# jhollowed/PyTEMDiags

Hardware: AMD Instinct MI355X
Metric: grid-points/sec through full TEM pipeline (ncol*nlev*nt) (higher is better)
Workload: dtype f64; 1 GPU; ne120 (777602 cols) x 72 lev x 30 snapshots per GPU, L=50, 1-degree zonal grid (M=180), ten GM16 Table-A1 outputs; ncol=777602, nlev=72, nt=30, sweeps=latitude-class, single sweep, mirror_paired_sweeps=True

## Files before the change

### include/temx.h

```cpp
#ifndef TEMX_H
#define TEMX_H

#include <stdint.h>

#ifdef __cplusplus
extern "C" {
#endif

typedef struct temx_plan temx_plan;

enum { TEMX_F64 = 0, TEMX_F32 = 1 };

enum {
  TEMX_OK = 0,
  TEMX_EINVAL = -1,
  TEMX_EHIP = -2,
  TEMX_ENOMEM = -3,
  TEMX_ERANK = -4,
  TEMX_ESTATE = -5,
  TEMX_EUNSUPPORTED = -6,
  TEMX_EINTERNAL = -7
};

enum {
  TEMX_DEFER_FINALIZE = 1,
  TEMX_NO_SYMMETRY = 2,
  TEMX_NO_CLASSES = 4,
  TEMX_NO_QR = 8,
  TEMX_LAT_TOL_F32 = 16
};

enum {
  TEMX_OPT_FORM = 1,
  TEMX_OPT_OS_MAP = 2,
  TEMX_OPT_OP_MAP = 3,
  TEMX_OPT_OS_SUBSAMPLE = 4,
  TEMX_OPT_TRACER_ONE_PASS = 5,
  TEMX_OPT_SINGLE_SWEEP_MIN_GROUPS = 6,
  TEMX_OPT_OS_CONTRACT = 7,
  TEMX_OPT_MISSING = 8,
  TEMX_OPT_MIN_COVERAGE = 9,
  TEMX_OPT_MISSING_WEIGHT = 10,
  TEMX_OPT_LAT_BINS = 12,
  TEMX_OPT_BIN_DEGREE = 13,
  TEMX_OPT_OS_SYNC = 11
};
enum {
  TEMX_FORM_AUTO = -1,
  TEMX_FORM_TWO_PASS = 0,
  TEMX_FORM_CLASS_SUMS = 1,
  TEMX_FORM_SINGLE_SWEEP = 2,
  TEMX_FORM_NO_SINGLE_SWEEP = 3,
  TEMX_FORM_MASKED = 4,
  TEMX_FORM_BINNED = 5
};

enum {
  TEMX_MAT_Y0 = 0,
  TEMX_MAT_Y0P = 1,
  TEMX_MAT_GRAM = 2,
  TEMX_MAT_GINV = 3,
  TEMX_MAT_Y0INV = 4,
  TEMX_MAT_GRAM2 = 5,
  TEMX_MAT_GX = 6,
  TEMX_MAT_GSUB = 7,
  TEMX_MAT_COVERAGE = 8
};
// ... 137 lines not shown
```

### pytemdiags_amd/_lib.py

```python
from __future__ import annotations

import ctypes as C
import os

_HERE = os.path.dirname(os.path.abspath(__file__))
LIB_PATH = os.environ.get("TEMX_LIB") or os.path.join(_HERE, "libtemx.so")

ABI_VERSION = 402
F64, F32 = 0, 1
DEFER_FINALIZE = 1
NO_SYMMETRY = 2
NO_CLASSES = 4
NO_QR = 8
LAT_TOL_F32 = 16
MAT_Y0, MAT_Y0P, MAT_GRAM, MAT_GINV, MAT_Y0INV, MAT_GRAM2, MAT_GX, MAT_GSUB = 0, 1, 2, 3, 4, 5, 6, 7
MAT_COVERAGE = 8
OPT_FORM, OPT_OS_MAP, OPT_OP_MAP, OPT_OS_SUBSAMPLE, OPT_TRACER_ONE_PASS, OPT_SINGLE_SWEEP_MIN_GROUPS, OPT_OS_CONTRACT = 1, 2, 3, 4, 5, 6, 7
OPT_MISSING, OPT_MIN_COVERAGE, OPT_MISSING_WEIGHT = 8, 9, 10
OPT_OS_SYNC = 11
OPT_LAT_BINS, OPT_BIN_DEGREE = 12, 13
LAT_BINS_ALLOWED = (128, 256, 512, 1024, 2048)
LAT_BINS_DEFAULT = 512
MISSING_MODES = {"raise": 0, "mask": 1}
FORM_AUTO, FORM_TWO_PASS, FORM_CLASS_SUMS, FORM_SINGLE_SWEEP, FORM_NO_SINGLE_SWEEP = -1, 0, 1, 2, 3
FORM_MASKED = 4
FORM_BINNED = 5
FORM_NAMES = {FORM_TWO_PASS: "two-pass", FORM_CLASS_SUMS: "class-sums", FORM_SINGLE_SWEEP: "single-sweep",
              FORM_MASKED: "masked", FORM_BINNED: "binned"}
FORMS = {"auto": FORM_AUTO, "two-pass": FORM_TWO_PASS, "class-sums": FORM_CLASS_SUMS,
         "single-sweep": FORM_SINGLE_SWEEP, "no-single-sweep": FORM_NO_SINGLE_SWEEP}

RESULT_NAMES = ("vtem", "omegatem", "wtem", "psitem", "epfy", "epfz", "epdiv",
                "utendepfd", "utendvtem", "utendwtem")
ZONAL_NAMES = ("ub", "vb", "thetab", "wapb", "upvpb", "upwappb", "vptpb", "dub_dp", "dthetab_dp",
               "ubcoslat", "dubcoslat_dlat", "psi", "psicoslat", "dpsicoslat_dlat", "dpsi_dp",
               "int_vbdp")
EDDY_NAMES = ("up", "vp", "thetap", "wapp", "upvp", "upwapp", "vptp")
TRACER_RESULT_NAMES = ("etfy", "etfz", "etdiv", "qtendetfd", "qtendvtem", "qtendwtem")
TRACER_ZONAL_NAMES = ("qb", "qpvpb", "qpwappb", "dqb_dp", "qbcoslat", "dqbcoslat_dlat")
TRACER_EDDY_NAMES = ("qp", "qpvp", "qpwapp")

ERRORS = {0: "TEMX_OK", -1: "TEMX_EINVAL", -2: "TEMX_EHIP", -3: "TEMX_ENOMEM", -4: "TEMX_ERANK",
          -5: "TEMX_ESTATE", -6: "TEMX_EUNSUPPORTED", -7: "TEMX_EINTERNAL"}
# ... 123 lines not shown
```

### pytemdiags_amd/csrc/kernels.hpp

```cpp
#pragma once
#include <hip/hip_runtime.h>
#include <stdint.h>

#include <type_traits>

#define TEMX_MFMA4(a, b, c) __builtin_amdgcn_mfma_f64_4x4x4f64((a), (b), (c), 0, 0, 0)

namespace temx {

template <int NF>
struct FieldPtrs {
  const void* p[NF];
};

struct EddyOut {
  double* p[7];
};

template <int KMAX>
__device__ __forceinline__ void basis_row(double xv, int K, const double* __restrict__ norm,
                                          const double* __restrict__ T, double* q) {
  double pm1 = 1.0, pc = xv;
  for (int l = 0; l < K; ++l) {
    double P;
// ... 220 lines not shown
#pragma unroll
    for (int j = 0; j < 16; ++j) t += sh[j][e];
    if (addend != nullptr) t += addend[idx];
    B[slice_index(map, idx)] = t;
    if (!(fabs(t) <= 1.79769313486231570815e308)) atomicOr(flag, 1);
  }
}

template <int NS>
__global__ void __launch_bounds__(256)
reduce_partials_flat_kernel(const double* __restrict__ partial, int nsplit, int64_t stride, int64_t n,
                            const double* __restrict__ addend, double* __restrict__ B, int* __restrict__ flag,
                            SliceMap map) {
  const int64_t idx = (int64_t)blockIdx.x * 256 + threadIdx.x;
  if (idx >= n) return;
  double v[NS];
#pragma unroll
  for (int sp = 0; sp < NS; ++sp) v[sp] = partial[(int64_t)(sp < nsplit ? sp : 0) * stride + idx];
  double t = 0.0;
#pragma unroll
  for (int sp = 0; sp < NS; ++sp) t += sp < nsplit ? v[sp] : 0.0;
  if (addend != nullptr) t += addend[idx];
  B[slice_index(map, idx)] = t;
  if (!(fabs(t) <= 1.79769313486231570815e308)) atomicOr(flag, 1);
}

__global__ void __launch_bounds__(256)
reduce_rows_kernel(const double* __restrict__ partial, int nsplit, int64_t stride, int nf, int rows_in, int rows,
                   int64_t D, double* __restrict__ out, int* __restrict__ flag) {
  const int64_t idx = (int64_t)blockIdx.x * 256 + threadIdx.x;
  const int64_t per = (int64_t)rows * D;
  if (idx >= per * nf) return;
  const int64_t f = idx / per, rem = idx - f * per;
  const double* src = partial + f * rows_in * D + rem;
  double t = 0.0;
  for (int sp = 0; sp < nsplit; ++sp) t += src[(int64_t)sp * stride];
  out[idx] = t;
  if (!(fabs(t) <= 1.79769313486231570815e308)) atomicOr(flag, 1);
}
__global__ void __launch_bounds__(256)
reduce_rows_wide_kernel(const double* __restrict__ partial, int nsplit, int64_t stride, int nf, int rows_in, int rows,
                        int64_t D, double* __restrict__ out, int* __restrict__ flag) {
  __shared__ double sh[16][17];
  const int e = threadIdx.x & 15, sl = threadIdx.x >> 4;
  const int64_t idx = (int64_t)blockIdx.x * 16 + e;
  const int64_t per = (int64_t)rows * D;
// ... 747 lines not shown
```

### pytemdiags_amd/csrc/kernels_op2.hpp

```cpp
#pragma once
#include "kernels_op.hpp"

namespace temx {

template <int NA, int NB>
struct OpwSlot {
  double sd[2][NA][64];
  double y[NB * 16];
};

template <int TBS, int NA>
__device__ __forceinline__ void opw_round(const OpwSlot<NA, 2 * TBS>* slots, int par, int t0, int nbw,
                                          uint32_t yoff, int lane, double (&acc)[NA][(TBS + 1) / 2]) {
  asm volatile("s_waitcnt lgkmcnt(0)\n\ts_barrier" ::: "memory");
#pragma unroll
  for (int j = 0; j < 4; ++j) {
    double b[NA];
#pragma unroll
    for (int f = 0; f < NA; ++f) b[f] = slots[j].sd[par][f][lane];
#pragma unroll
    for (int tl = 0; tl < (TBS + 1) / 2; ++tl)
      if (tl < nbw) {
        const double ya = slots[j].y[(t0 + tl) * 16 + yoff];
#pragma unroll
// ... 937 lines not shown
    }
    if (hfail != 0 && lane == 0) atomicOr(hstat, hfail);
  }
  if (left > 0) {
    const int first = (b1 - b0) & (NCH - 1);
    static_for<NCH>([&](auto cc) __attribute__((always_inline)) {
      if (((decltype(cc)::value - first) & (NCH - 1)) < left) pending_chunk(cc);
    });
  }
  if (dvalid) {
#pragma unroll
    for (int f = 0; f < NFX; ++f)
#pragma unroll
      for (int t = 0; t < NBX; ++t) {
        const int l = symx_harm<TBX>(t, g);
        if (l < (pp != nullptr ? KX : K4)) px[(((int64_t)split * NFX + f) * KX + l) * D + d] = ax[f][t];
      }
#pragma unroll
    for (int k = 0; k < NP; ++k)
#pragma unroll
      for (int t = 0; t < 2 * TBS; ++t) {
        const int l = sym_harm<TBS>(t, g);
        if (pp != nullptr && l < K) pp[(((int64_t)split * NP + k) * K + l) * D + d] = k < NPR ? apr[k < NPR ? k : 0][t] : apl[((k < NPR ? 0 : k - NPR) * 2 * TBS + t) * 64];
      }
  }
}

#ifndef TEMX_OS2_STAGGER
#define TEMX_OS2_STAGGER 0
#endif
#ifndef TEMX_OS2_ACC32
#define TEMX_OS2_ACC32 1
#endif
template <typename T, int TBS, int TBX, int NBR, int PD, int KIND = 0>
__global__ void __launch_bounds__(512, 1)
sweep_os2_kernel(FieldPtrs<4> fp, int64_t D, int K, int KX, const double* __restrict__ ycx,
                 const int4* __restrict__ crowN, const int4* __restrict__ crowS,
                 const int* __restrict__ gfirstN, const int* __restrict__ gfirstS, const int2* __restrict__ csplit,
                 const double* __restrict__ colscale, const double* __restrict__ rho, int K4,
                 double* __restrict__ px, double* __restrict__ pp, int nsplit, int ndt) {
  using KD = OsKind<KIND>;
  constexpr int NF = KD::NF, NFX = KD::NFX, NP = KD::NP;
  constexpr int NBX = 2 * TBX;
  constexpr int YE = NBX * 16;
  constexpr int MB = CLS_MB;
  constexpr int NCH = 2;
// ... 500 lines not shown
}

__global__ void __launch_bounds__(256)
os_ref_solve_kernel(const double* __restrict__ As, int KX , int KR, int64_t D,
                    const double* __restrict__ Gsinv, double* __restrict__ rho) {
  __shared__ double sg[16 * 16];
  const int f = blockIdx.y;
  for (int i = threadIdx.x; i < KR * KR; i += blockDim.x) sg[i] = Gsinv[i];
  __syncthreads();
  const int64_t d = blockIdx.x * (int64_t)(blockDim.x / 16) + (threadIdx.x & 15);
  const int l = threadIdx.x >> 4;
  if (d >= D || l >= KR) return;
  const double* a = As + (int64_t)f * KX * D + d;
  double v0 = 0.0, v1 = 0.0;
  int m = 0;
  for (; m + 2 <= KR; m += 2) {
    v0 += sg[l * KR + m] * a[(int64_t)m * D];
    v1 += sg[l * KR + m + 1] * a[(int64_t)(m + 1) * D];
  }
  if (m < KR) v0 += sg[l * KR + m] * a[(int64_t)m * D];
  rho[((int64_t)f * KR + l) * D + d] = v0 + v1;
}

constexpr int OSC = 4;
constexpr int OSR = 256 / OSC;

__device__ __forceinline__ void os_stage(double* dst, const double* __restrict__ src, int n, int tid) {
  for (int i = tid; i < n; i += 256) dst[i] = src[i];
}

__host__ __device__ inline size_t os_contract_lds(int K, int KX, int NQ) {
  const size_t big = (size_t)NQ * KX > (size_t)2 * K * K ? (size_t)NQ * KX : (size_t)2 * K * K;
  return ((size_t)4 * KX + 8 * K + 8 * NQ + 3 * KX + 3 * K) * OSC + big;
}

struct OsFields {
  const double* A[4];
  const double* rho[4];
};

template <int KIND>
__global__ void __launch_bounds__(256)
os_contract_kernel(OsFields in, const double* __restrict__ Pp,
                   int K, int KX, int KR, int NQ, int64_t D, const double* __restrict__ Tm,
                   const double* __restrict__ G2inv, const double* __restrict__ G, const double* __restrict__ Gx,
                   const double* __restrict__ Yq, const double* __restrict__ wq2, double* __restrict__ B4,
// ... 144 lines not shown
```

### pytemdiags_amd/csrc/temx.hip

```cpp
#include "../../include/temx.h"
#include "../../include/temx_vert.h"
#include "../../include/temx_layout.h"
#include "../../include/temx_ingest.h"
#include "../../include/temx_clim.h"
#include "../../include/temx_mtracer.h"
#include "../../include/temx_nclim.h"
#include "../../include/temx_gclim.h"
#include "../include/temx_mgclim.h"
#include "../include/temx_wave.h"
#include "../include/temx_tfilt.h"

#include <hip/hip_runtime.h>

#include <algorithm>
#include <cmath>
#include <cstdarg>
#include <cstdio>
#include <cstdlib>
#include <cstring>
#include <map>
#include <mutex>
#include <new>
#include <stdexcept>
#include <string>
// ... 125 lines not shown
  std::vector<int> gbatch0;
  DevBuf crow, ycls;
  std::map<int, DevBuf> csplits;
  Split sp_cproj4, sp_cproj1, sp_ceddy, sp_cflux;
  bool os_built = false, os_on = false;
  bool os_valid = false;
  DevBuf Axq, rho_t;
  int TBX = 0, KX = 0, KR = 0, NQ = 0;
  std::vector<double> h_xc, h_cnt;
  std::vector<int> h_crow;
  std::vector<int> sgbatch0;
  int64_t sgroups = 0, sbatches = 0;
  DevBuf ycx, ycx_s, crow_s, rho, rho0, gaunt , wq2, Gx, Gsinv, Ax , Axs ;
  std::vector<double> h_G_own;
  std::vector<double> h_Gx_own;
  std::vector<double> h_Gx, h_Gs;
  std::vector<double> h_T, h_Ginv, h_G, h_Yq;
  DevBuf oscblk, osAt, osAb, osAtq, osAbq, Bqp;
  OscMats osc{};
  bool osc_lds = false;
  int opt_os_contract = -1;
  bool os_barrier = false;
  int opt_os_sync = -1;
  int os_keep = 32;
  int64_t tD = 0, tnt = 0, tt0 = 0;
  int opt_form = -1, opt_os_map = -1, opt_op_map = -1, opt_tracer_one_pass = -1, opt_single_sweep_min_groups = -1;
  bool os_tile = false, op_tile = false;
  bool no_qr = false;
  DevBuf side_crow[2][2], side_gfirst[2][2];
  std::map<int, DevBuf> csplits_s;
  Split sp_os, sp_os_s;
  Split sp_copw;
  bool lcls = false, lone = false, xb_valid = false;
  DevBuf ycls_l, pbuf;
  int64_t ycls_lstride = 0;
  Split sp_lflux;
  bool onepass = false, op_valid = false;
  bool c4_valid = false;
  DevBuf csum, ccnt;
  DevBuf Pq;
  DevBuf csq, Pq2;
  bool tq_valid = false;
  DevBuf partial;
  DevBuf opB, opC;
  int opt_missing = 0, opt_min_cov = 500, opt_miss_w = 10;
  bool miss_built = false;
// ... 168 lines not shown
}

static int launch_reduce(temx_plan* pl, const double* partial, int nsplit, int64_t n, double* B,
                         hipStream_t st, int64_t stride = -1, const double* addend = nullptr,
                         const SliceMap& map = SliceMap(), int* flag = nullptr) {
  if (stride < 0) stride = n;
  if (flag == nullptr) flag = static_cast<int*>(pl->flag.p);
  if (nsplit <= 16 && n >= 32768) {
    const dim3 grid((unsigned)((n + 255) / 256));
    if (nsplit <= 2)
      hipLaunchKernelGGL(reduce_partials_flat_kernel<2>, grid, dim3(256), 0, st, partial, nsplit, stride, n, addend, B, flag, map);
    else if (nsplit <= 4)
      hipLaunchKernelGGL(reduce_partials_flat_kernel<4>, grid, dim3(256), 0, st, partial, nsplit, stride, n, addend, B, flag, map);
    else if (nsplit <= 8)
      hipLaunchKernelGGL(reduce_partials_flat_kernel<8>, grid, dim3(256), 0, st, partial, nsplit, stride, n, addend, B, flag, map);
    else
      hipLaunchKernelGGL(reduce_partials_flat_kernel<16>, grid, dim3(256), 0, st, partial, nsplit, stride, n, addend, B, flag, map);
    HIPCHK(hipGetLastError());
    return TEMX_OK;
  }
  const int64_t blocks = (n + 15) / 16;
  hipLaunchKernelGGL(reduce_partials_kernel, dim3((unsigned)blocks), dim3(256), 0, st, partial, nsplit, stride, n,
                     addend, B, flag, map);
  HIPCHK(hipGetLastError());
  return TEMX_OK;
}

static int launch_reduce_rows(temx_plan* pl, const double* partial, int nsplit, int64_t stride, int nf, int rows_in,
                              int rows, int64_t D, double* out, hipStream_t st) {
  const int64_t n = (int64_t)nf * rows * D;
  if (nsplit > 16)
    hipLaunchKernelGGL(reduce_rows_wide_kernel, dim3((unsigned)((n + 15) / 16)), dim3(256), 0, st, partial, nsplit, stride,
                       nf, rows_in, rows, D, out, static_cast<int*>(pl->flag.p));
  else
    hipLaunchKernelGGL(reduce_rows_kernel, dim3((unsigned)((n + 255) / 256)), dim3(256), 0, st, partial, nsplit, stride,
                       nf, rows_in, rows, D, out, static_cast<int*>(pl->flag.p));
  HIPCHK(hipGetLastError());
  return TEMX_OK;
}

static int launch_solve(temx_plan* pl, const double* B, int NF, int64_t D, double* C, double* Xb,
                        hipStream_t st) {
  if (pl->K <= 64) {
    const int nmb = (pl->M + 3) / 4;
    const int gx = (int)(((D + 15) / 16 + 3) / 4);
    int mbs = SOLVE_MB;
// ... 472 lines not shown
          static_cast<const int*>(pl->side_gfirst[si][0].p), static_cast<const int*>(pl->side_gfirst[si][1].p),
          cuts, pl->colscale.d(), rho, pl->KR, px, pp, sp.nsplit, sp.ndt);
    }
    constexpr size_t lds = sweep_osr_lds(TBSv, TBXv, KD::NF, KD::NP, KD::NPR, DF);
    static_assert(lds <= 163840, "the single sweep's workgroup fits the LDS of a compute unit");
    auto go = [&](auto handoff) {
      return launch_lds<sweep_osr_kernel<double, TBSv, TBXv, NBR, 2, KIND, decltype(handoff)::value>>(pl->device, grid,
          block, lds, st, fp, pl->D, pl->K, pl->KX, sub ? pl->ycx_s.d() : pl->ycx.d(),
          static_cast<const int4*>(sub ? pl->crow_s.p : pl->crow.p), cuts, pl->colscale.d(), rho, pl->KR, px, pp, sp.nsplit,
          sp.ndt, static_cast<int*>(pl->flag.p) + 1);
    };
    return pl->os_barrier ? go(Int<0>{}) : go(Int<1>{});
  });
  return listed ? rc : fail(TEMX_EUNSUPPORTED, "single-sweep form: no instantiation for L = %d", pl->L);
}

template <int KIND>
static int launch_sweep_os(temx_plan* pl, const FieldPtrs<4>& fp, int dtype, bool sub, const double* rho, double* partial,
                           const Split& sp, hipStream_t st) {
  return dtype == TEMX_F64 ? launch_sweep_os_t<double, KIND>(pl, fp, sub, rho, partial, sp, st)
                           : launch_sweep_os_t<float, KIND>(pl, fp, sub, rho, partial, sp, st);
}

static bool os_supported(const temx_plan* pl) {
  return os_supported(pl->cls, pl->large, pl->weighted, pl->qbasis, !pl->h_crow.empty(), pl->TBS, pl->L);
}

static bool os_active(const temx_plan* pl, int dtype) {
  (void)dtype;
  return pl->os_on;
}

static void set_tail(temx_plan* pl, int64_t t0, int64_t nts) {
  if (pl->tt0 != t0 || pl->tnt != nts) pl->c4_valid = pl->os_valid = pl->op_valid = pl->tq_valid = pl->xb_valid = false;
  pl->tt0 = t0;
  pl->tnt = nts;
  pl->tD = (int64_t)pl->nlev * nts;
}
static inline bool tail_is_whole(const temx_plan* pl) { return pl->tt0 == 0 && pl->tnt == pl->nt; }

static int tem_stage3_impl(temx_plan* pl, const double* B3, double* results, double* zonal, hipStream_t st);
static int tem_epilogue(temx_plan* pl, double* results, double* zonal, hipStream_t st);
static int bin_project_op(temx_plan* pl, const void* A, int dtype, int64_t D, double* B, hipStream_t st);
static int bin_zonal_mean(temx_plan* pl, const void* A, int dtype, int64_t D, double* out, int native, hipStream_t st);
static int miss_check(const temx_plan* pl);
static int miss_zonal_mean(temx_plan* pl, const void* A, int dtype, int64_t D, double* out, int native, hipStream_t st);
// ... 10 lines not shown
  return m;
}

template <int NBK>
static int launch_osc_t(temx_plan* pl, const OscFieldsIn& fin, int nf, int nout, double* Bf, double* At, double* ab,
                        const OscPairsIn& pin, int np, double* Bp, int64_t Dt, hipStream_t st) {
  const unsigned gx = (unsigned)((Dt + 15) / 16);
  hipLaunchKernelGGL((osc_fields_kernel<NBK>), dim3(gx, nf, 2), dim3(OSC_W * 64), (size_t)osc_fields_lds(NBK) * 8, st, fin, pl->osc, pl->K,
                     pl->KX, pl->KR, pl->NQ, Dt, nout, Bf, At, ab, pl->D, (int)pl->tnt, (int)pl->nt, (int)pl->tt0);
  HIPCHK(hipGetLastError());
  hipLaunchKernelGGL((osc_pairs_kernel<NBK>), dim3(gx, np), dim3(OSC_W * 64), (size_t)osc_pairs_lds(NBK) * 8, st, pin, pl->osc, pl->wq2.d(),
                     pl->K, pl->KX, pl->NQ, Dt, Bp);
  HIPCHK(hipGetLastError());
  return TEMX_OK;
}
static int launch_osc(temx_plan* pl, const OscFieldsIn& fin, int nf, int nout, double* Bf, double* At, double* ab,
                      const OscPairsIn& pin, int np, double* Bp, int64_t Dt, hipStream_t st) {
  if (pl->TB == 13 && pl->TBX == 13) return launch_osc_t<13>(pl, fin, nf, nout, Bf, At, ab, pin, np, Bp, Dt, st);
  if (pl->TB == 8 && pl->TBX == 8) return launch_osc_t<8>(pl, fin, nf, nout, Bf, At, ab, pin, np, Bp, Dt, st);
  if (pl->TB == 4 && pl->TBX == 4) return launch_osc_t<4>(pl, fin, nf, nout, Bf, At, ab, pin, np, Bp, Dt, st);
  return fail(TEMX_EUNSUPPORTED, "single-sweep contraction: no instantiation for L = %d", pl->L);
}

static int os_prepass(temx_plan* pl, const FieldPtrs<4>& fp, int dtype, double* As, hipStream_t st) {
  int rc;
  const int64_t D = pl->D, KD4 = (int64_t)4 * pl->KX * D;
  pl->op_valid = pl->c4_valid = pl->tq_valid = pl->os_valid = false;
  if ((rc = launch_sweep_os<0>(pl, fp, dtype, true, pl->rho0.d(), pl->partial.d(), pl->sp_os_s, st))) return rc;
  return launch_reduce_rows(pl, pl->partial.d(), pl->sp_os_s.nsplit, KD4, 4, pl->KX, pl->KR, D, As, st);
}

static int os_sweep(temx_plan* pl, const FieldPtrs<4>& fp, int dtype, const double* As, int nsl, double* proj, hipStream_t st) {
  int rc;
  const int64_t D = pl->D;
  const int64_t KD4 = (int64_t)4 * pl->KX * D, KD3 = (int64_t)3 * pl->K * D;
  pl->op_valid = pl->c4_valid = pl->tq_valid = pl->os_valid = false;
  hipLaunchKernelGGL(os_ref_solve_kernel, dim3((unsigned)((D + 15) / 16), 4), dim3(256), 0, st, As, pl->KR, pl->KR, D,
                     pl->Gsinv.d(), pl->rho.d());
  HIPCHK(hipGetLastError());
  TimedLaunch tl{};
  time_begin(pl, 0, st, tl);
  rc = launch_sweep_os<0>(pl, fp, dtype, false, pl->rho.d(), pl->partial.d(), pl->sp_os, st);
  time_end(pl, 0, st, tl);
  if (rc) return rc;
  const int64_t rows = (int64_t)4 * pl->KX + 3 * pl->K;
  if ((rc = launch_reduce(pl, pl->partial.d(), pl->sp_os.nsplit, KD4, proj, st, -1, nullptr, slice_map(pl, nsl, rows, 0)))) return rc;
  return launch_reduce(pl, pl->partial.d() + (int64_t)pl->sp_os.nsplit * KD4, pl->sp_os.nsplit, KD3, nsl > 1 ? proj : proj + KD4, st, -1,
                       nullptr, slice_map(pl, nsl, rows, (int64_t)4 * pl->KX));
}

static int os_tail(temx_plan* pl, const double* proj_s, int64_t t0, int64_t nts, double* results, double* zonal, hipStream_t st) {
  int rc;
  set_tail(pl, t0, nts);
  const int64_t Dt = pl->tD;
  const int64_t rows = (int64_t)4 * pl->KX + 3 * pl->K;
  if (proj_s != pl->Ax.d())
    HIPCHK(hipMemcpyAsync(pl->Ax.p, proj_s, (size_t)rows * Dt * 8, hipMemcpyDeviceToDevice, st));
  {
    TimedLaunch t2{};
    time_begin(pl, 1, st, t2);
    const size_t lds = os_contract_lds(pl->K, pl->KX, pl->NQ) * 8;
    const double* Pp = pl->Ax.d() + (int64_t)4 * pl->KX * Dt;
    if (pl->osc_lds) {
      OsFields in;
      for (int f = 0; f < 4; ++f) {
        in.A[f] = pl->Ax.d() + (int64_t)f * pl->KX * Dt;
        in.rho[f] = pl->rho.d() + (int64_t)f * pl->KR * pl->D;
      }
// ... 9 lines not shown
      for (int f = 0; f < 4; ++f) {
        fin.A[f] = pl->Ax.d() + (int64_t)f * pl->KX * Dt;
        fin.rho[f] = pl->rho.d() + (int64_t)f * pl->KR * pl->D;
      }
      for (int k = 0; k < 3; ++k) {
        pin.At_a[k] = pl->osAt.d() + KD::pa(k) * QD; pin.At_b[k] = pl->osAt.d() + KD::pb(k) * QD;
        pin.ab_a[k] = pl->osAb.d() + KD::pa(k) * QD; pin.ab_b[k] = pl->osAb.d() + KD::pb(k) * QD;
        pin.P[k] = Pp + (int64_t)k * pl->K * Dt;
      }
      if ((rc = launch_osc(pl, fin, 4, 4, pl->B4.d(), pl->osAt.d(), pl->osAb.d(), pin, 3, pl->B3.d(), Dt, st))) return rc;
    }
    time_end(pl, 1, st, t2);
  }
  if ((rc = launch_solve(pl, pl->B4.d(), 4, Dt, pl->C4.d(), pl->zb.d(), st))) return rc;
  if ((rc = tem_stage3_impl(pl, pl->B3.d(), results, zonal, st))) return rc;
  pl->c4_valid = true;
  pl->os_valid = true;
  return TEMX_OK;
}

static int tem_run_os(temx_plan* pl, const FieldPtrs<4>& fp, int dtype, double* results, double* zonal, void* stream) {
  hipStream_t st = S_(stream);
  int rc;
  if ((rc = os_prepass(pl, fp, dtype, pl->Axs.d(), st))) return rc;
  if ((rc = os_sweep(pl, fp, dtype, pl->Axs.d(), 1, pl->Ax.d(), st))) return rc;
  return os_tail(pl, pl->Ax.d(), 0, pl->nt, results, zonal, st);
}

static int tracer_ws(temx_plan* pl);

static int tracer_os_ws(temx_plan* pl, int nq) {
  const TracerOsWs w = tracer_os_ws_layout(tem_dims(pl), nq, pl->KX, pl->KR, pl->NQ);
  int rc;
  if ((rc = tracer_ws(pl))) return rc;
  if ((rc = pl->Axq.ensure(w.Axq))) return rc;
  if ((rc = pl->osAtq.ensure(w.osAtq))) return rc;
  if ((rc = pl->osAbq.ensure(w.osAbq))) return rc;
  if ((rc = pl->Bqp.ensure(w.Bqp))) return rc;
  return pl->rho_t.ensure(w.rho_t);
}

static int tracer_os_prepass(temx_plan* pl, int nq, const FieldPtrs<4>& fp, int dtype, double* Asq, hipStream_t st) {
  int rc;
  const int64_t D = pl->D;
  if ((rc = tracer_os_ws(pl, nq))) return rc;
  pl->tq_valid = false;
  rc = nq == 2 ? launch_sweep_os<3>(pl, fp, dtype, true, pl->rho0.d(), pl->partial.d(), pl->sp_os_s, st)
               : launch_sweep_os<1>(pl, fp, dtype, true, pl->rho0.d(), pl->partial.d(), pl->sp_os_s, st);
// ... 1225 lines not shown
      break;
    case TEMX_OPT_MISSING_WEIGHT:
      if (value < 4 || value > 14) return fail(TEMX_EINVAL, "TEMX_OPT_MISSING_WEIGHT: tau = 10^-value, value in 4..14, got %d", value);
      pl->opt_miss_w = value;
      break;
    case TEMX_OPT_OS_SYNC:
      if (value != 0 && value != 1) return fail(TEMX_EINVAL, "TEMX_OPT_OS_SYNC: 0 (flags) or 1 (barriers), got %d", value);
      pl->opt_os_sync = value;
      break;
    case TEMX_OPT_LAT_BINS: {
      const int B = value == -1 ? BIN_DEFAULT : value;
      if (B != 0) {
        if (!bin_count_ok(B)) return fail(TEMX_EINVAL, "TEMX_OPT_LAT_BINS: 0 (off), -1 (default, %d) or one of 128, 256, 512, 1024, 2048, got %d", BIN_DEFAULT, value);
        if (int rc = bin_check(pl)) return rc;
        if (bin_degree(pl->L, B) == 0)
          return fail(TEMX_EINVAL, "TEMX_OPT_LAT_BINS: (L, B) = (%d, %d): no Chebyshev degree up to %d keeps the basis rows to %.0e; use more bins",
                      pl->L, B, BIN_MAX_DEGREE, BIN_BOUND);
      }
      pl->opt_lat_bins = B;
      pl->bin_J = B ? bin_degree(pl->L, B) : 0;
      break;
    }
    case TEMX_OPT_BIN_DEGREE: return fail(TEMX_EINVAL, "TEMX_OPT_BIN_DEGREE is chosen by the library (read it with temx_plan_option)");
    default: return fail(TEMX_EINVAL, "unknown option %d", option);
  }
  pl->tem = false;
  return TEMX_OK;
} TEMX_CATCH

int temx_plan_option(const temx_plan* pl, int option) try {
  if (!pl) return -1;
  switch (option) {
    case TEMX_OPT_FORM:
      if (miss_mode(pl)) return TEMX_FORM_MASKED;
      if (bin_mode(pl)) return TEMX_FORM_BINNED;
      return pl->os_on ? TEMX_FORM_SINGLE_SWEEP : ((pl->cls && pl->onepass) || (pl->lcls && pl->lone) ? TEMX_FORM_CLASS_SUMS : TEMX_FORM_TWO_PASS);
    case TEMX_OPT_OS_MAP: return tile_map(pl->opt_os_map, "TEMX_OS_MAP") ? 1 : 0;
    case TEMX_OPT_OP_MAP: return tile_map(pl->opt_op_map, "TEMX_OP_MAP") ? 1 : 0;
    case TEMX_OPT_TRACER_ONE_PASS: return tracer_one_pass_wanted(pl) ? 1 : 0;
    case TEMX_OPT_OS_SUBSAMPLE: return pl->os_keep;
    case TEMX_OPT_SINGLE_SWEEP_MIN_GROUPS: return pl->opt_single_sweep_min_groups;
    case TEMX_OPT_OS_CONTRACT: return pl->osc_lds ? 1 : 0;
    case TEMX_OPT_MISSING: return pl->opt_missing;
    case TEMX_OPT_MIN_COVERAGE: return pl->opt_min_cov;
    case TEMX_OPT_MISSING_WEIGHT: return pl->opt_miss_w;
    case TEMX_OPT_OS_SYNC: return os_barrier_wanted(pl) ? 1 : 0;
    case TEMX_OPT_LAT_BINS: return pl->opt_lat_bins;
    case TEMX_OPT_BIN_DEGREE: return pl->bin_J;
    default: return -1;
  }
} TEMX_CATCH

static bool mem_free(size_t* fr) {
  size_t tot = 0;
  return hipMemGetInfo(fr, &tot) == hipSuccess;
}

static int set_tem_large_cls(temx_plan* pl, const TemDims& d, const FormChoice& fc) {
  const LargeClsLayout l = tem_large_cls_layout(d, fc);
  size_t fr = 0;
  if (!(l.eligible && mem_free(&fr) && fits(l.csum, pl->csum.bytes, fr, l.pbuf) &&
        alloc_write_stream(pl->csum, l.csum) == TEMX_OK && pl->pbuf.ensure(l.pbuf) == TEMX_OK))
    return TEMX_OK;
  int rc;
  HIPCHK(hipMemset(pl->csum.p, 0, pl->csum.bytes));
  HIPCHK(hipMemset(pl->pbuf.p, 0, pl->pbuf.bytes));
  pl->sp_cproj4 = l.sp_cproj4;
  pl->sp_cflux = l.sp_cflux;
  pl->sp_lflux = l.sp_lflux;
  if ((rc = pl->partial.ensure(l.partial))) return rc;
  if ((rc = pl->Bs.ensure(l.Bs))) return rc;
// ... 1721 lines not shown
```

### pytemdiags_amd/engine.py

```python
from __future__ import annotations

import ctypes as C

import numpy as np
import torch

from . import _lib
from ._lib import check

_DT = {torch.float64: _lib.F64, torch.float32: _lib.F32}


def _ptr(t):
    return C.c_void_p(t.data_ptr())


def _dbl(a):
    a = np.ascontiguousarray(a, dtype=np.float64)
    return a, a.ctypes.data_as(C.POINTER(C.c_double))


def lat_bins_value(lat_bins):
    if lat_bins is None or lat_bins is False:
        return 0
# ... 33 lines not shown

    @property
    def paired(self):
        return bool(self.lib.temx_plan_is_paired(self._h))

    @property
    def sweep_mode(self):
        return int(self.lib.temx_plan_sweep_mode(self._h))

    @property
    def one_pass(self):
        return bool(self.lib.temx_plan_one_pass(self._h))

    @property
    def single_sweep(self):
        return bool(self.lib.temx_plan_single_sweep(self._h))

    @property
    def tracer_one_pass(self):
        return self.one_pass and self.option(_lib.OPT_TRACER_ONE_PASS) == 1

    def configure(self, form=None, os_map=None, op_map=None, os_subsample=None, tracer_one_pass=None,
                  single_sweep_min_groups=None, os_contract=None, missing=None, min_coverage=None,
                  missing_weight=None, os_sync=None, lat_bins=None):
        def put(opt, val):
            check(self.lib.temx_plan_configure(self._h, opt, int(val)))
        if missing is not None:
            if missing not in _lib.MISSING_MODES:
                raise ValueError("missing must be 'raise' or 'mask', got %r" % (missing,))
            put(_lib.OPT_MISSING, _lib.MISSING_MODES[missing])
        if min_coverage is not None:
            mc = float(min_coverage)
            if not 0.0 <= mc <= 1.0:
                raise ValueError("min_coverage must lie in [0, 1], got %r" % (min_coverage,))
            put(_lib.OPT_MIN_COVERAGE, int(round(mc * 1000)))
        if missing_weight is not None:
            e = -np.log10(float(missing_weight))
            if not (float(missing_weight) > 0 and abs(e - round(e)) < 1e-9 and 4 <= round(e) <= 14):
                raise ValueError("missing_weight must be 10^-n with n in 4..14, got %r" % (missing_weight,))
            put(_lib.OPT_MISSING_WEIGHT, int(round(e)))
        if form is not None:
            put(_lib.OPT_FORM, _lib.FORMS[form] if isinstance(form, str) else form)
            self.form_requested = form
        for opt, val in ((_lib.OPT_OS_MAP, os_map), (_lib.OPT_OP_MAP, op_map)):
            if val is not None:
                put(opt, {"row": 0, "tile": 1}[val] if isinstance(val, str) else val)
        if os_subsample is not None:
            put(_lib.OPT_OS_SUBSAMPLE, os_subsample)
        if tracer_one_pass is not None:
# ... 681 lines not shown
```

Measured before the change: 189.2 billion grid-points/s.

## Add lean single-sweep pre-pass kernel and merge reduce/solve launches

Adds a specialized pre-pass kernel that computes only the four-field zonal-mean projections, replacing the general single-sweep kernel on the f64 untiled path. The partial reduction is fused with the reference solve so the separate solve launch is skipped. The two partial reductions after the main sweep are merged into one flat launch. Together these aim to cut launch count and redundant work in the chain, at the cost of more kernel code and a new option that lets users restore the old chain.

After: 188.5 billion grid-points/s (median of 2 runs). No clear change (-0.3%).

```diff
diff --git a/include/temx.h b/include/temx.h
--- a/include/temx.h
+++ b/include/temx.h
@@ -43,6 +43,7 @@
   TEMX_OPT_MISSING_WEIGHT = 10,
   TEMX_OPT_LAT_BINS = 12,
   TEMX_OPT_BIN_DEGREE = 13,
+  TEMX_OPT_OS_CHAIN = 14,
   TEMX_OPT_OS_SYNC = 11
 };
 enum {
diff --git a/pytemdiags_amd/_lib.py b/pytemdiags_amd/_lib.py
--- a/pytemdiags_amd/_lib.py
+++ b/pytemdiags_amd/_lib.py
@@ -19,6 +19,7 @@
 OPT_MISSING, OPT_MIN_COVERAGE, OPT_MISSING_WEIGHT = 8, 9, 10
 OPT_OS_SYNC = 11
 OPT_LAT_BINS, OPT_BIN_DEGREE = 12, 13
+OPT_OS_CHAIN = 14
 LAT_BINS_ALLOWED = (128, 256, 512, 1024, 2048)
 LAT_BINS_DEFAULT = 512
 MISSING_MODES = {"raise": 0, "mask": 1}
diff --git a/pytemdiags_amd/csrc/kernels.hpp b/pytemdiags_amd/csrc/kernels.hpp
--- a/pytemdiags_amd/csrc/kernels.hpp
+++ b/pytemdiags_amd/csrc/kernels.hpp
@@ -266,6 +266,27 @@
   for (int sp = 0; sp < NS; ++sp) t += sp < nsplit ? v[sp] : 0.0;
   if (addend != nullptr) t += addend[idx];
   B[slice_index(map, idx)] = t;
+  if (!(fabs(t) <= 1.79769313486231570815e308)) atomicOr(flag, 1);
+}
+
+template <int NS>
+__global__ void __launch_bounds__(256)
+reduce_partials_flat2_kernel(const double* __restrict__ p1, int64_t n1, double* __restrict__ B1,
+                             const double* __restrict__ p2, int64_t n2, double* __restrict__ B2, int nsplit,
+                             int* __restrict__ flag) {
+  const int64_t nb1 = (n1 + 255) / 256;
+  const bool second = (int64_t)blockIdx.x >= nb1;
+  const int64_t idx = ((int64_t)blockIdx.x - (second ? nb1 : 0)) * 256 + threadIdx.x;
+  const int64_t n = second ? n2 : n1;
+  if (idx >= n) return;
+  const double* __restrict__ partial = second ? p2 : p1;
+  double v[NS];
+#pragma unroll
+  for (int sp = 0; sp < NS; ++sp) v[sp] = partial[(int64_t)(sp < nsplit ? sp : 0) * n + idx];
+  double t = 0.0;
+#pragma unroll
+  for (int sp = 0; sp < NS; ++sp) t += sp < nsplit ? v[sp] : 0.0;
+  (second ? B2 : B1)[idx] = t;
   if (!(fabs(t) <= 1.79769313486231570815e308)) atomicOr(flag, 1);
 }
 
diff --git a/pytemdiags_amd/csrc/kernels_op2.hpp b/pytemdiags_amd/csrc/kernels_op2.hpp
--- a/pytemdiags_amd/csrc/kernels_op2.hpp
+++ b/pytemdiags_amd/csrc/kernels_op2.hpp
@@ -983,6 +983,192 @@
       for (int t = 0; t < 2 * TBS; ++t) {
         const int l = sym_harm<TBS>(t, g);
         if (pp != nullptr && l < K) pp[(((int64_t)split * NP + k) * K + l) * D + d] = k < NPR ? apr[k < NPR ? k : 0][t] : apl[((k < NPR ? 0 : k - NPR) * 2 * TBS + t) * 64];
+      }
+  }
+}
+
+template <typename T, int TBX, int NBR, int PD>
+__global__ void __launch_bounds__(256, 2)
+sweep_osr_pre_kernel(FieldPtrs<4> fp, int64_t D, int KX, const double* __restrict__ ycx,
+                     const int4* __restrict__ crow, const int2* __restrict__ csplit,
+                     const double* __restrict__ colscale, int K4, double* __restrict__ px, int nsplit, int ndt) {
+  using KD = OsKind<0>;
+  constexpr int NF = KD::NF;
+  constexpr int NBX = 2 * TBX;
+  constexpr int YE = NBX * 16;
+  constexpr int MB = CLS_MB;
+  constexpr int NB4 = 2 * NBR;
+  constexpr int NV = 2 * NF;
+  static_assert(NBR <= TBX && NB4 == 4, "row_wait has a form for four Y operands");
+  static_assert((PD - 1) * MB * NF + (MB - 1) * NF <= 63 && PD <= CLS_PADB - 1, "the ring is counted in vmcnt (6 bits)");
+  static_assert(PD == 4, "the wait for the Y operands names one count per batch issued since");
+  __shared__ double lds[16 + NV * 256];
+  int split, dq;
+  if (!wg_work((ndt + 3) / 4, nsplit, split, dq)) return;
+  const int tid = threadIdx.x;
+  const int wave = uniform_wave(), lane = tid & 63;
+  const int c = lane & 15, g = lane >> 4;
+  const int64_t colr = (int64_t)dq * 64 + lane < D ? (int64_t)dq * 64 + lane : D - 1;
+  const uint32_t colb32 = (uint32_t)colr * (uint32_t)sizeof(T);
+  const int dt = dq * 4 + wave;
+  const int64_t d = (int64_t)dt * 16 + c;
+  const bool dvalid = dt < ndt && d < D;
+  const int b0 = __builtin_amdgcn_readfirstlane(csplit[split].x);
+  const int b1 = __builtin_amdgcn_readfirstlane(csplit[split + 1].x);
+  int grp = __builtin_amdgcn_readfirstlane(csplit[split].y);
+  const uint32_t aoff_p = (uint32_t)(g * 4 + (lane & 3));
+  double* cn = lds;
+  double* ex = lds + 16;
+  double* exw = ex + wave * 64 + lane;
+  const double* exr = ex + g * 64 + wave * 16 + c;
+  const double sth = colscale != nullptr ? colscale[colr] : 1.0;
+  uint64_t fbase[NF];
+#pragma unroll
+  for (int f = 0; f < NF; ++f) fbase[f] = reinterpret_cast<uint64_t>(fp.p[f]);
+  { double sth_ready = sth; asm volatile("" : "+v"(sth_ready)); }
+
+  double ax[NF][NB4];
+#pragma unroll
+  for (int f = 0; f < NF; ++f)
+#pragma unroll
+    for (int t = 0; t < NB4; ++t) ax[f][t] = 0.0;
+  double s[NF], x0[NF], cnt = 0.0;
+  double sN[NF], x0N[NF], cntN = 0.0;
+#pragma unroll
+  for (int f = 0; f < NF; ++f) s[f] = x0[f] = sN[f] = x0N[f] = 0.0;
+  bool north_open = false, prev_south = false;
+  const uint32_t rowbytes = (uint32_t)D * (uint32_t)sizeof(T);
+
+  T xb[PD][MB][NF];
+  int er[PD][MB];
+  double ya[NB4];
+  int since = PD;
+  uint32_t yoff32[NB4];
+#pragma unroll
+  for (int t = 0; t < NB4; ++t) yoff32[t] = (uint32_t)((t < NBR ? t : TBX + (t - NBR)) * 16 + (int)aoff_p) * 8u;
+  auto load_ya = [&](int gi) __attribute__((always_inline)) {
+#pragma unroll
+    for (int t = 0; t < NB4; ++t) RowLoad<double>::ld(ya[t], yoff32[t], reinterpret_cast<uint64_t>(ycx) + (uint64_t)gi * (YE * 8));
+    since = 0;
+  };
+  auto issue = [&](auto pc, const int4 rv) __attribute__((always_inline)) {
+    constexpr int P = decltype(pc)::value;
+    er[P][0] = rv.x; er[P][1] = rv.y; er[P][2] = rv.z; er[P][3] = rv.w;
+#pragma unroll
+    for (int j = 0; j < MB; ++j) {
+      const uint64_t off = (uint64_t)(uint32_t)(er[P][j] & CLS_ROWMASK) * rowbytes;
+#pragma unroll
+      for (int f = 0; f < NF; ++f) RowLoad<T>::ld(xb[P][j][f], colb32, fbase[f] + off);
+    }
+  };
+  auto park_north = [&]() __attribute__((always_inline)) {
+#pragma unroll
+    for (int f = 0; f < NF; ++f) { sN[f] = s[f]; x0N[f] = x0[f]; s[f] = 0.0; }
+    cntN = cnt;
+    cnt = 0.0;
+  };
+  int4 rn;
+  auto step = [&](auto posc, int b) __attribute__((always_inline)) {
+    constexpr int P = decltype(posc)::value % PD;
+    {
+      const int4 r1 = rn;
+      rn = crow[(int64_t)(b + PD) * 4 + wave];
+      issue(std::integral_constant<int, (P + PD - 1) % PD>{}, r1);
+      ++since;
+    }
+    static_for<MB>([&](auto jc) __attribute__((always_inline)) {
+      constexpr int j = decltype(jc)::value;
+      constexpr int NW = (PD - 1) * MB * NF + (MB - 1 - j) * NF;
+      row_wait<NW>(xb[P][j][0], xb[P][j][1], xb[P][j][2], xb[P][j][3]);
+    });
+    const int fl = er[P][0] >> 27;
+    const bool south = (fl & (CLS_SOUTH << 1)) != 0;
+    if ((fl & (CLS_FIRST << 1)) || (south && !prev_south)) {
+      if (south && north_open) park_north();
+      north_open = !south;
+#pragma unroll
+      for (int f = 0; f < NF; ++f) x0[f] = (double)xb[P][0][f];
+    }
+    prev_south = south;
+#pragma unroll
+    for (int j = 0; j < MB; ++j) {
+      const double w = er[P][j] < 0 ? 0.0 : 1.0;
+      double dx[NF];
+#pragma unroll
+      for (int f = 0; f < NF; ++f) dx[f] = (double)xb[P][j][f] - x0[f];
+#pragma unroll
+      for (int f = 0; f < NF; ++f) s[f] += w * dx[f];
+      cnt += w;
+    }
+    if (fl & (CLS_LAST << 1)) {
+      prev_south = false;
+      if (north_open) park_north();
+      north_open = false;
+      const double rnN = cntN > 0.0 ? temx_rcp_count(cntN) : 0.0, rnS = cnt > 0.0 ? temx_rcp_count(cnt) : 0.0;
+      double val[NV];
+#pragma unroll
+      for (int f = 0; f < NF; ++f) {
+        const double sc = f == KD::TF ? sth : 1.0;
+        val[f] = (sN[f] * rnN + x0N[f]) * sc;
+        val[NF + f] = (s[f] * rnS + x0[f]) * sc;
+      }
+      asm volatile("s_waitcnt lgkmcnt(0)\n\ts_barrier" ::: "memory");
+#pragma unroll
+      for (int v = 0; v < NV; ++v) exw[v * 256] = val[v];
+      if (lane == 0) {
+        cn[wave] = cntN;
+        cn[4 + wave] = cnt;
+      }
+      asm volatile("s_waitcnt lgkmcnt(0)\n\ts_barrier" ::: "memory");
+      const double nN = cn[g], nS = cn[4 + g];
+      double dS[NF][2];
+#pragma unroll
+      for (int f = 0; f < NF; ++f) {
+        const double SNf = nN * exr[f * 256], SSf = nS * exr[(NF + f) * 256];
+        dS[f][0] = SNf + SSf;
+        dS[f][1] = SNf - SSf;
+      }
+      if (since == 1) row_wait<MB * NF>(ya[0], ya[1], ya[2], ya[3]);
+      else if (since == 2) row_wait<2 * MB * NF>(ya[0], ya[1], ya[2], ya[3]);
+      else if (since == 3) row_wait<3 * MB * NF>(ya[0], ya[1], ya[2], ya[3]);
+#pragma unroll
+      for (int t = 0; t < NB4; ++t) row_touch(ya[t]);
+#pragma unroll
+      for (int t = 0; t < NB4; ++t)
+#pragma unroll
+        for (int f = 0; f < NF; ++f) ax[f][t] = TEMX_MFMA4(ya[t], dS[f][t < NBR ? 0 : 1], ax[f][t]);
+      ++grp;
+      load_ya(grp);
+#pragma unroll
+      for (int f = 0; f < NF; ++f) s[f] = sN[f] = 0.0;
+      cnt = cntN = 0.0;
+    }
+  };
+
+  if (b0 < b1) {
+    load_ya(grp);
+    since = PD;
+    rn = crow[(int64_t)b0 * 4 + wave];
+    static_for<PD - 1>([&](auto kc) __attribute__((always_inline)) {
+      constexpr int k = decltype(kc)::value;
+      const int4 r0 = rn;
+      rn = crow[(int64_t)(b0 + k + 1) * 4 + wave];
+      issue(kc, r0);
+    });
+    for (int b = b0; b < b1; b += PD)
+      static_for<PD>([&](auto kc) __attribute__((always_inline)) {
+        constexpr int k = decltype(kc)::value;
+        if (k == 0 || b + k < b1) step(kc, b + k);
+      });
+    asm volatile("s_waitcnt vmcnt(0)" ::: "memory");
+  }
+  if (dvalid) {
+#pragma unroll
+    for (int f = 0; f < NF; ++f)
+#pragma unroll
+      for (int t = 0; t < NB4; ++t) {
+        const int l = t < NBR ? 2 * (4 * t + g) : 2 * (4 * (t - NBR) + g) + 1;
+        if (l < K4) px[(((int64_t)split * NF + f) * KX + l) * D + d] = ax[f][t];
       }
   }
 }
@@ -1529,6 +1715,38 @@
   rho[((int64_t)f * KR + l) * D + d] = v0 + v1;
 }
 
+__global__ void __launch_bounds__(256)
+os_reduce_ref_solve_kernel(const double* __restrict__ partial, int nsplit, int64_t stride, int rows_in, int KR, int64_t D,
+                           const double* __restrict__ Gsinv, double* __restrict__ As, double* __restrict__ rho,
+                           int* __restrict__ flag) {
+  __shared__ double sg[16 * 16];
+  __shared__ double sa[16][16];
+  const int f = blockIdx.y;
+  for (int i = threadIdx.x; i < KR * KR; i += blockDim.x) sg[i] = Gsinv[i];
+  const int dl = threadIdx.x & 15;
+  const int64_t d = blockIdx.x * (int64_t)16 + dl;
+  const int l = threadIdx.x >> 4;
+  const bool mine = d < D && l < KR;
+  if (mine) {
+    const double* src = partial + ((int64_t)f * rows_in + l) * D + d;
+    double t = 0.0;
+    for (int sp = 0; sp < nsplit; ++sp) t += src[(int64_t)sp * stride];
+    As[((int64_t)f * KR + l) * D + d] = t;
+    if (!(fabs(t) <= 1.79769313486231570815e308)) atomicOr(flag, 1);
+    sa[l][dl] = t;
+  }
+  __syncthreads();
+  if (!mine) return;
+  double v0 = 0.0, v1 = 0.0;
+  int m = 0;
+  for (; m + 2 <= KR; m += 2) {
+    v0 += sg[l * KR + m] * sa[m][dl];
+    v1 += sg[l * KR + m + 1] * sa[m + 1][dl];
+  }
+  if (m < KR) v0 += sg[l * KR + m] * sa[m][dl];
+  rho[((int64_t)f * KR + l) * D + d] = v0 + v1;
+}
+
 constexpr int OSC = 4;
 constexpr int OSR = 256 / OSC;
 
diff --git a/pytemdiags_amd/csrc/temx.hip b/pytemdiags_amd/csrc/temx.hip
--- a/pytemdiags_amd/csrc/temx.hip
+++ b/pytemdiags_amd/csrc/temx.hip
@@ -171,6 +171,7 @@
   int opt_os_contract = -1;
   bool os_barrier = false;
   int opt_os_sync = -1;
+  int opt_os_chain = 0;
   int os_keep = 32;
   int64_t tD = 0, tnt = 0, tt0 = 0;
   int opt_form = -1, opt_os_map = -1, opt_op_map = -1, opt_tracer_one_pass = -1, opt_single_sweep_min_groups = -1;
@@ -385,6 +386,22 @@
   const int64_t blocks = (n + 15) / 16;
   hipLaunchKernelGGL(reduce_partials_kernel, dim3((unsigned)blocks), dim3(256), 0, st, partial, nsplit, stride, n,
                      addend, B, flag, map);
+  HIPCHK(hipGetLastError());
+  return TEMX_OK;
+}
+
+static int launch_reduce_two(temx_plan* pl, const double* p1, int64_t n1, double* B1, const double* p2, int64_t n2, double* B2,
+                             int nsplit, hipStream_t st) {
+  const dim3 grid((unsigned)((n1 + 255) / 256 + (n2 + 255) / 256));
+  int* flag = static_cast<int*>(pl->flag.p);
+  if (nsplit <= 2)
+    hipLaunchKernelGGL(reduce_partials_flat2_kernel<2>, grid, dim3(256), 0, st, p1, n1, B1, p2, n2, B2, nsplit, flag);
+  else if (nsplit <= 4)
+    hipLaunchKernelGGL(reduce_partials_flat2_kernel<4>, grid, dim3(256), 0, st, p1, n1, B1, p2, n2, B2, nsplit, flag);
+  else if (nsplit <= 8)
+    hipLaunchKernelGGL(reduce_partials_flat2_kernel<8>, grid, dim3(256), 0, st, p1, n1, B1, p2, n2, B2, nsplit, flag);
+  else
+    hipLaunchKernelGGL(reduce_partials_flat2_kernel<16>, grid, dim3(256), 0, st, p1, n1, B1, p2, n2, B2, nsplit, flag);
   HIPCHK(hipGetLastError());
   return TEMX_OK;
 }
@@ -903,6 +920,18 @@
                            : launch_sweep_os_t<float, KIND>(pl, fp, sub, rho, partial, sp, st);
 }
 
+static int launch_sweep_os_pre(temx_plan* pl, const FieldPtrs<4>& fp, double* partial, const Split& sp, hipStream_t st) {
+  const int2* cuts = nullptr;
+  if (int rc = os_cuts_dev(pl, true, sp.nsplit, &cuts)) return rc;
+  int rc = TEMX_OK;
+  const bool listed = dispatch_strict(OsPairs{}, pl->TBS, pl->TBX, rc, [&](auto pair) {
+    constexpr int TBXv = decltype(pair)::second;
+    return launch<sweep_osr_pre_kernel<double, TBXv, OS_NBR, 4>>(dim3(sp.grid), dim3(256), 0, st, fp, pl->D, pl->KX,
+        pl->ycx_s.d(), static_cast<const int4*>(pl->crow_s.p), cuts, pl->colscale.d(), pl->KR, partial, sp.nsplit, sp.ndt);
+  });
+  return listed ? rc : fail(TEMX_EUNSUPPORTED, "single-sweep form: no instantiation for L = %d", pl->L);
+}
+
 static bool os_supported(const temx_plan* pl) {
   return os_supported(pl->cls, pl->large, pl->weighted, pl->qbasis, !pl->h_crow.empty(), pl->TBS, pl->L);
 }
@@ -959,28 +988,48 @@
   return fail(TEMX_EUNSUPPORTED, "single-sweep contraction: no instantiation for L = %d", pl->L);
 }
 
-static int os_prepass(temx_plan* pl, const FieldPtrs<4>& fp, int dtype, double* As, hipStream_t st) {
+static int os_prepass(temx_plan* pl, const FieldPtrs<4>& fp, int dtype, double* As, hipStream_t st, bool* with_rho = nullptr) {
   int rc;
   const int64_t D = pl->D, KD4 = (int64_t)4 * pl->KX * D;
   pl->op_valid = pl->c4_valid = pl->tq_valid = pl->os_valid = false;
-  if ((rc = launch_sweep_os<0>(pl, fp, dtype, true, pl->rho0.d(), pl->partial.d(), pl->sp_os_s, st))) return rc;
+  const bool lean = pl->opt_os_chain == 0;
+  if (lean && dtype == TEMX_F64 && !pl->os_tile)
+    rc = launch_sweep_os_pre(pl, fp, pl->partial.d(), pl->sp_os_s, st);
+  else
+    rc = launch_sweep_os<0>(pl, fp, dtype, true, pl->rho0.d(), pl->partial.d(), pl->sp_os_s, st);
+  if (rc) return rc;
+  if (with_rho != nullptr) {
+    *with_rho = lean && pl->sp_os_s.nsplit <= 16;
+    if (*with_rho) {
+      hipLaunchKernelGGL(os_reduce_ref_solve_kernel, dim3((unsigned)((D + 15) / 16), 4), dim3(256), 0, st, pl->partial.d(),
+                         pl->sp_os_s.nsplit, KD4, pl->KX, pl->KR, D, pl->Gsinv.d(), As, pl->rho.d(), static_cast<int*>(pl->flag.p));
+      HIPCHK(hipGetLastError());
+      return TEMX_OK;
+    }
+  }
   return launch_reduce_rows(pl, pl->partial.d(), pl->sp_os_s.nsplit, KD4, 4, pl->KX, pl->KR, D, As, st);
 }
 
-static int os_sweep(temx_plan* pl, const FieldPtrs<4>& fp, int dtype, const double* As, int nsl, double* proj, hipStream_t st) {
+static int os_sweep(temx_plan* pl, const FieldPtrs<4>& fp, int dtype, const double* As, int nsl, double* proj, hipStream_t st,
+                    bool have_rho = false) {
   int rc;
   const int64_t D = pl->D;
   const int64_t KD4 = (int64_t)4 * pl->KX * D, KD3 = (int64_t)3 * pl->K * D;
   pl->op_valid = pl->c4_valid = pl->tq_valid = pl->os_valid = false;
-  hipLaunchKernelGGL(os_ref_solve_kernel, dim3((unsigned)((D + 15) / 16), 4), dim3(256), 0, st, As, pl->KR, pl->KR, D,
-                     pl->Gsinv.d(), pl->rho.d());
-  HIPCHK(hipGetLastError());
+  if (!have_rho) {
+    hipLaunchKernelGGL(os_ref_solve_kernel, dim3((unsigned)((D + 15) / 16), 4), dim3(256), 0, st, As, pl->KR, pl->KR, D,
+                       pl->Gsinv.d(), pl->rho.d());
+    HIPCHK(hipGetLastError());
+  }
   TimedLaunch tl{};
   time_begin(pl, 0, st, tl);
   rc = launch_sweep_os<0>(pl, fp, dtype, false, pl->rho.d(), pl->partial.d(), pl->sp_os, st);
   time_end(pl, 0, st, tl);
   if (rc) return rc;
   const int64_t rows = (int64_t)4 * pl->KX + 3 * pl->K;
+  if (nsl <= 1 && pl->opt_os_chain == 0 && pl->sp_os.nsplit <= 16 && KD3 >= 32768 && KD4 >= 32768)
+    return launch_reduce_two(pl, pl->partial.d(), KD4, proj, pl->partial.d() + (int64_t)pl->sp_os.nsplit * KD4, KD3, proj + KD4,
+                             pl->sp_os.nsplit, st);
   if ((rc = launch_reduce(pl, pl->partial.d(), pl->sp_os.nsplit, KD4, proj, st, -1, nullptr, slice_map(pl, nsl, rows, 0)))) return rc;
   return launch_reduce(pl, pl->partial.d() + (int64_t)pl->sp_os.nsplit * KD4, pl->sp_os.nsplit, KD3, nsl > 1 ? proj : proj + KD4, st, -1,
                        nullptr, slice_map(pl, nsl, rows, (int64_t)4 * pl->KX));
@@ -1036,8 +1085,9 @@
 static int tem_run_os(temx_plan* pl, const FieldPtrs<4>& fp, int dtype, double* results, double* zonal, void* stream) {
   hipStream_t st = S_(stream);
   int rc;
-  if ((rc = os_prepass(pl, fp, dtype, pl->Axs.d(), st))) return rc;
-  if ((rc = os_sweep(pl, fp, dtype, pl->Axs.d(), 1, pl->Ax.d(), st))) return rc;
+  bool have_rho = false;
+  if ((rc = os_prepass(pl, fp, dtype, pl->Axs.d(), st, &have_rho))) return rc;
+  if ((rc = os_sweep(pl, fp, dtype, pl->Axs.d(), 1, pl->Ax.d(), st, have_rho))) return rc;
   return os_tail(pl, pl->Ax.d(), 0, pl->nt, results, zonal, st);
 }
 
@@ -2309,6 +2359,10 @@
       break;
     }
     case TEMX_OPT_BIN_DEGREE: return fail(TEMX_EINVAL, "TEMX_OPT_BIN_DEGREE is chosen by the library (read it with temx_plan_option)");
+    case TEMX_OPT_OS_CHAIN:
+      if (value != 0 && value != 1) return fail(TEMX_EINVAL, "TEMX_OPT_OS_CHAIN: 0 (pre-pass kernel, merged launches) or 1 (the earlier chain), got %d", value);
+      pl->opt_os_chain = value;
+      return TEMX_OK;
     default: return fail(TEMX_EINVAL, "unknown option %d", option);
   }
   pl->tem = false;
@@ -2334,6 +2388,7 @@
     case TEMX_OPT_OS_SYNC: return os_barrier_wanted(pl) ? 1 : 0;
     case TEMX_OPT_LAT_BINS: return pl->opt_lat_bins;
     case TEMX_OPT_BIN_DEGREE: return pl->bin_J;
+    case TEMX_OPT_OS_CHAIN: return pl->opt_os_chain;
     default: return -1;
   }
 } TEMX_CATCH
diff --git a/pytemdiags_amd/engine.py b/pytemdiags_amd/engine.py
--- a/pytemdiags_amd/engine.py
+++ b/pytemdiags_amd/engine.py
@@ -79,9 +79,14 @@
 
     def configure(self, form=None, os_map=None, op_map=None, os_subsample=None, tracer_one_pass=None,
                   single_sweep_min_groups=None, os_contract=None, missing=None, min_coverage=None,
-                  missing_weight=None, os_sync=None, lat_bins=None):
+                  missing_weight=None, os_sync=None, lat_bins=None, os_chain=None):
         def put(opt, val):
             check(self.lib.temx_plan_configure(self._h, opt, int(val)))
+        if os_chain is not None:
+            put(_lib.OPT_OS_CHAIN, {"merged": 0, "separate": 1}[os_chain] if isinstance(os_chain, str) else os_chain)
+            if all(v is None for v in (form, os_map, op_map, os_subsample, tracer_one_pass, single_sweep_min_groups,
+                                       os_contract, missing, min_coverage, missing_weight, os_sync, lat_bins)):
+                return
         if missing is not None:
             if missing not in _lib.MISSING_MODES:
                 raise ValueError("missing must be 'raise' or 'mask', got %r" % (missing,))
```
